# aws/s2n-quic

Measured on AMD Instinct MI355X. Metric: GiB/s AEAD seal+open, device-resident, 1200 B packets at 1/2/4/8 MI355X, higher is better.
Workload: dtype u8

## Files before the change

### s2n-quic_amd/csrc/check_resources.py

```python
import re
import sys

bad = []
for path in sys.argv[1:]:
    name = None
    for line in open(path, errors="replace"):
        m = re.search(r"remark: Function Name: (\S+)", line)
        if m:
            name = m.group(1)
            continue
        if not name:
            continue
        lds = re.search(r"LDS Size \[bytes/block\]: (\d+)", line)
        scr = re.search(r"ScratchSize \[bytes/lane\]: (\d+)", line)
        dyn_lds = any(k in name for k in ("aes_gcm_quad_kernel", "aes_gcm_quad_rx_kernel", "aes_gcm_wave_kernel",
                                          "aes_gcm_burst_kernel", "txq_server_kernel"))
        default = ("aes_gcm_wave_kernel" in name or re.search(r"aes_gcm_quad_kernelILb[01]ELi10E", name)
                   or re.search(r"aes_gcm_quad_rx_kernelILi10E", name))
        if lds and dyn_lds and int(lds.group(1)) != 0:
            bad.append(f"{name}: {lds.group(1)} B of static LDS on top of the dynamic 160 KiB")
        if scr and default and int(scr.group(1)) > 32:
            bad.append(f"{name}: {scr.group(1)} B/lane of scratch")
if bad:
    sys.exit("kernel resource check failed:\n  " + "\n  ".join(bad))
```

### s2n-quic_amd/csrc/device_common.h

```cpp
#pragma once

#include <utility>

#include "qpp_internal.h"

namespace qpp {
namespace dev {

constexpr uint32_t kLdsGhash = 0;
constexpr uint32_t kLdsAes = 65536;
constexpr uint32_t kLdsV = 131072;
constexpr uint32_t kLdsStage = 131072;
constexpr uint32_t kLdsMax = 163840;

typedef uint32_t u32x4 __attribute__((ext_vector_type(4)));
typedef __attribute__((address_space(3))) uint32_t lds_u32;
typedef __attribute__((address_space(3))) u32x4 lds_u128;
__device__ __forceinline__ uint32_t lds_ld32(uint32_t a) { return *(const lds_u32 *)(size_t)a; }
__device__ __forceinline__ uint4 lds_ld128(uint32_t a) {
    const u32x4 v = *(const lds_u128 *)(size_t)a;
    return make_uint4(v.x, v.y, v.z, v.w);
}
__device__ __forceinline__ void lds_st32(uint32_t a, uint32_t v) { *(lds_u32 *)(size_t)a = v; }
__device__ __forceinline__ uint32_t lds_add32(uint32_t a, uint32_t v) {
// ... 374 lines not shown
    const uint32_t s = d_sbox[x], s2 = xtime4(s);
    const uint32_t t0 = s2 | (s << 8) | (s << 16) | ((s2 ^ s) << 24);
    for (uint32_t d = threadIdx.x; d < 8192; d += blockDim.x) {
        const uint32_t slot = ((d >> 8) + x) & 31u, m = slot >> 3;
        lds_st32(base + 256u * x + 4u * slot, __builtin_amdgcn_alignbit(t0, t0, (32u - 8u * m) & 31u));
    }
}

#ifdef __HIP_DEVICE_COMPILE__
typedef const __attribute__((address_space(4))) uint4 *RkPtr;
#else
typedef const uint4 *RkPtr;
#endif

struct CtrPageQ4 {
    uint32_t k0, k1, k2, k3;
    uint32_t l0, l1, l2, l3;
    uint32_t x3;
    uint32_t page;

    template <typename RK>
    __device__ __forceinline__ void build(const AesQ4 &a, RK rkp, uint32_t n0, uint32_t n1, uint32_t n2, uint32_t pg) {
        const uint4 r0 = rkp[0], r1 = rkp[1], r2 = rkp[2];
        const uint32_t rk[12] = {r0.x, r0.y, r0.z, r0.w, r1.x, r1.y, r1.z, r1.w, r2.x, r2.y, r2.z, r2.w};
        build(a, rk, n0, n1, n2, pg);
    }
    __device__ __forceinline__ void build(const AesQ4 &a, const uint32_t *__restrict__ rk, uint32_t n0, uint32_t n1,
                                          uint32_t n2, uint32_t pg) {
        const uint32_t s0 = a.rot(n0 ^ rk[0]), s1 = a.rot(n1 ^ rk[1]), s2 = a.rot(n2 ^ rk[2]),
                       s3 = a.rot(bswap32(pg << 8) ^ rk[3]);
        k0 = xor3(a.look<0>(s0), a.look<1>(s1), a.look<2>(s2)) ^ a.rot(rk[4]);
        k1 = a.col(s1, s2, s3, s0, a.rot(rk[5]));
        k2 = a.col(s2, s3, s0, s1, a.rot(rk[6]));
        k3 = a.col(s3, s0, s1, s2, a.rot(rk[7]));
        l0 = xor3(a.look<1>(k1), a.look<2>(k2), a.look<3>(k3)) ^ a.rot(rk[8]);
        l1 = xor3(a.look<0>(k1), a.look<1>(k2), a.look<2>(k3)) ^ a.rot(rk[9]);
        l2 = xor3(a.look<0>(k2), a.look<1>(k3), a.look<3>(k1)) ^ a.rot(rk[10]);
        l3 = xor3(a.look<0>(k3), a.look<2>(k1), a.look<3>(k2)) ^ a.rot(rk[11]);
        x3 = rk[3] >> 24;
        page = pg;
    }
    __device__ __forceinline__ void two_rounds(const AesQ4 &a, uint32_t c, uint32_t (&v)[4]) const {
        const uint32_t u0 = k0 ^ a.lookx(c ^ x3);
        v[0] = l0 ^ a.look<0>(u0);
        v[1] = l1 ^ a.look<3>(u0);
        v[2] = l2 ^ a.look<2>(u0);
        v[3] = l3 ^ a.look<1>(u0);
    }
};

#ifndef QPP_Q4_DEPTH
#define QPP_Q4_DEPTH 3
#endif
template <int NR, int NB, int STRIDE = 1>
__device__ __forceinline__ void ctr_keystream_q4(const AesQ4 &a, const CtrPageQ4 &pg, const uint32_t *__restrict__ rk,
                                                 uint32_t c0, uint4 (&ks)[NB]) {
    static_assert(NB >= 1 && NB <= 4, "pipeline depth NB - 1 lookups groups of 4 within the 15-read counter");
    constexpr int D = NB - 1 < QPP_Q4_DEPTH ? NB - 1 : QPP_Q4_DEPTH;
    constexpr int U = (NR - 2) * 4 * NB;
    uint32_t st[NB][4];
    uint32_t nw[4];
    uint32_t kr[4];
    uint32_t ld[D + 1][4];
#pragma unroll
    for (int j = 0; j < NB; j++) pg.two_rounds(a, c0 + STRIDE * j, st[j]);
    auto issue = [&](auto uc) {
        constexpr int u = decltype(uc)::value;
        constexpr int j = (u / 4) % NB, c = u % 4;
        const uint32_t *s = st[j];
        uint32_t *l = ld[u % (D + 1)];
        l[0] = a.look<0>(s[c]);
        l[1] = a.look<1>(s[(c + 1) & 3]);
        l[2] = a.look<2>(s[(c + 2) & 3]);
        l[3] = a.look<3>(s[(c + 3) & 3]);
    };
    auto combine = [&](auto uc) {
        constexpr int u = decltype(uc)::value;
        constexpr int r = 3 + u / (4 * NB), j = (u / 4) % NB, c = u % 4;
        const uint32_t *l = ld[u % (D + 1)];
        if constexpr (u % (4 * NB) == 0) {
#pragma unroll
            for (int i = 0; i < 4; i++) kr[i] = r < NR ? a.rot(rk[4 * r + i]) : rk[4 * r + i];
        }
        if constexpr (r < NR) {
            nw[c] = AesQ4::comb(l[0], l[1], l[2], l[3], kr[c]);
        } else {
            nw[c] = a.fin(l[0], l[1], l[2], l[3], kr[c]);
        }
        if constexpr (c == 3) {
#pragma unroll
            for (int i = 0; i < 4; i++) st[j][i] = nw[i];
        }
    };
    static_for<D>([&](auto uc) { issue(uc); });
    static_for<U>([&](auto uc) {
        constexpr int u = decltype(uc)::value;
        if constexpr (u + D < U) issue(std::integral_constant<int, u + D>{});
        __builtin_amdgcn_sched_barrier(0);
        combine(uc);
        __builtin_amdgcn_sched_barrier(0);
    });
#pragma unroll
    for (int j = 0; j < NB; j++) ks[j] = make_uint4(st[j][0], st[j][1], st[j][2], st[j][3]);
}

struct PacketView {
    uint8_t *base;
    uint32_t aad_len, len, pn_len;
    uint32_t n0, n1, n2;
};

// ... 225 lines not shown
```

### s2n-quic_amd/csrc/ghash.h

```cpp
#pragma once

#include "device_common.h"

namespace qpp {
namespace dev {

#ifndef QPP_GHASH_DEPTH
#define QPP_GHASH_DEPTH 9
#endif
template <bool PIPE>
struct GhashT {
    uint32_t lc[4];
    uint32_t sel[4];
    bool q1, q2;

    __device__ __forceinline__ static GhashT make() {
        GhashT g;
        const uint32_t r = threadIdx.x & 15u, q = r >> 2, b = r & 3u;
#pragma unroll
        for (int k = 0; k < 4; k++) {
            uint32_t v = 0;
#pragma unroll
            for (int i = 0; i < 4; i++) v |= ((4u * ((k + q) & 3u) + ((i + b) & 3u)) << 4) << (8 * i);
            g.lc[k] = v;
        }
#pragma unroll
        for (int i = 0; i < 4; i++) g.sel[i] = 0x0c0c0000u | ((4u + ((i + b) & 3u)) << 8) | (uint32_t)i;
        g.q1 = q & 1u;
        g.q2 = (q >> 1) & 1u;
        return g;
    }
    __device__ __forceinline__ uint4 rot(uint4 z) const {
        const uint4 a = q1 ? make_uint4(z.y, z.z, z.w, z.x) : z;
        return q2 ? make_uint4(a.z, a.w, a.x, a.y) : a;
    }
    template <int K, int I>
    __device__ __forceinline__ uint4 look(const uint4 &w) const {
        const uint32_t wk = K == 0 ? w.x : K == 1 ? w.y : K == 2 ? w.z : w.w;
        return lds_ld128(kLdsGhash + __builtin_amdgcn_perm(wk, lc[K], sel[I]));
    }
    __device__ __forceinline__ uint4 prod(const uint4 &w, uint4 c) const {
        if constexpr (!PIPE) {
            const uint4 a = xor3(look<0, 0>(w), look<0, 1>(w), look<0, 2>(w));
            const uint4 b = xor3(look<0, 3>(w), look<1, 0>(w), look<1, 1>(w));
            const uint4 d = xor3(look<1, 2>(w), look<1, 3>(w), look<2, 0>(w));
            const uint4 e = xor3(look<2, 1>(w), look<2, 2>(w), look<2, 3>(w));
            const uint4 f = xor3(look<3, 0>(w), look<3, 1>(w), look<3, 2>(w));
            const uint4 g = xor3(a, b, d);
            const uint4 h = xor3(e, f, look<3, 3>(w));
            return xor3(g, h, c);
        }
        if constexpr (QPP_GHASH_DEPTH != 9) return prod_d<QPP_GHASH_DEPTH>(w, c);
        uint4 l[16];
        auto issue = [&](auto ic) {
            constexpr int i = decltype(ic)::value;
            l[i] = look<i / 4, i % 4>(w);
        };
        static_for<9>(issue);
        __builtin_amdgcn_sched_barrier(0);
        const uint4 a = xor3(l[0], l[1], l[2]);
        issue(std::integral_constant<int, 9>{});
        issue(std::integral_constant<int, 10>{});
        issue(std::integral_constant<int, 11>{});
        __builtin_amdgcn_sched_barrier(0);
        const uint4 b = xor3(l[3], l[4], l[5]);
        issue(std::integral_constant<int, 12>{});
        issue(std::integral_constant<int, 13>{});
        issue(std::integral_constant<int, 14>{});
        __builtin_amdgcn_sched_barrier(0);
        const uint4 d = xor3(l[6], l[7], l[8]);
        issue(std::integral_constant<int, 15>{});
        __builtin_amdgcn_sched_barrier(0);
        const uint4 g = xor3(a, b, d);
        const uint4 e = xor3(l[9], l[10], l[11]);
        const uint4 f = xor3(l[12], l[13], l[14]);
        const uint4 h = xor3(e, f, l[15]);
        return xor3(g, h, c);
    }
    template <int D>
    __device__ __forceinline__ uint4 prod_d(const uint4 &w, uint4 c) const {
        uint4 l[16], x[5];
        auto issue = [&](auto ic) {
            constexpr int i = decltype(ic)::value;
            if constexpr (i < 16) l[i] = look<i / 4, i % 4>(w);
        };
        static_for<D>(issue);
        static_for<5>([&](auto tc) {
            constexpr int t = decltype(tc)::value;
            __builtin_amdgcn_sched_barrier(0);
            x[t] = xor3(l[3 * t], l[3 * t + 1], l[3 * t + 2]);
            issue(std::integral_constant<int, 3 * t + D>{});
            issue(std::integral_constant<int, 3 * t + D + 1>{});
            issue(std::integral_constant<int, 3 * t + D + 2>{});
        });
        __builtin_amdgcn_sched_barrier(0);
        return xor3(xor3(x[0], x[1], x[2]), xor3(x[3], x[4], l[15]), c);
    }
    __device__ __forceinline__ uint4 mulx(const uint4 &w, uint4 c) const { return rot(prod(w, c)); }
};
using Ghash = GhashT<false>;

__device__ inline void build_tables(const DevKey *__restrict__ key) {
    const uint32_t tid = threadIdx.x, nthr = blockDim.x;
    for (uint32_t i = tid; i < 128; i += nthr) {
        const uint32_t *v = key->V[i];
        lds_st128(kLdsV + 16 * i, make_uint4(v[0], v[1], v[2], v[3]));
    }
    build_aes_tables(kLdsAes);
    __syncthreads();
    for (uint32_t e = tid; e < 4096; e += nthr) {
        const uint32_t j = e & 15, x = e >> 4;
        uint4 acc = make_uint4(0, 0, 0, 0);
#pragma unroll
        for (int i = 0; i < 8; i++)
            if ((x >> (7 - i)) & 1) acc = acc ^ lds_ld128(kLdsV + 16 * (8 * j + i));
        lds_st128(kLdsGhash + 256 * x + 16 * j, acc);
    }
    __syncthreads();
}

template <uint32_t BASE = kLdsGhash>
struct Ghash4T {
    Ghash g;
    uint32_t hi_or, lo_or;
    __device__ __forceinline__ static Ghash4T make(uint32_t wave) {
        Ghash4T h;
        h.g = Ghash::make();
        h.hi_or = 0x01010101u * ((2u * wave + 0u) << 4);
        h.lo_or = 0x01010101u * ((2u * wave + 1u) << 4);
        return h;
    }
    __device__ __forceinline__ uint4 rot(uint4 z) const { return g.rot(z); }
    template <int K, int I>
    __device__ __forceinline__ uint4 look(uint32_t wk) const {
        return lds_ld128(BASE + __builtin_amdgcn_perm(wk, g.lc[K], g.sel[I]));
    }
    __device__ __forceinline__ uint4 prod(const uint4 &w, uint4 c) const { return prod_impl<true>(w, c); }
    __device__ __forceinline__ uint4 prod(const uint4 &w) const { return prod_impl<false>(w, w); }
    template <bool C>
    __device__ __forceinline__ uint4 prod_impl(const uint4 &w, uint4 c) const {
        const uint32_t wk[4] = {w.x, w.y, w.z, w.w};
        uint32_t hs[4], ls[4];
#pragma unroll
        for (int k = 0; k < 4; k++) {
            hs[k] = __builtin_amdgcn_bitop3_b32(wk[k] >> 4, 0x0f0f0f0fu, hi_or, 0xea);
            ls[k] = __builtin_amdgcn_bitop3_b32(wk[k], 0x0f0f0f0fu, lo_or, 0xea);
        }
        uint4 r[32];
        auto issue = [&](auto ic) {
// ... 44 lines not shown
```

### s2n-quic_amd/csrc/quad.hip

```cpp
#include <stdlib.h>

#include "device_common.h"
#include "ghash.h"

namespace qpp {
namespace {
using namespace dev;

constexpr uint32_t kQLdsPow = 131072;
constexpr uint32_t kQLdsVe = 65536;
#ifndef QPP_QUAD_WG
#define QPP_QUAD_WG 768
#endif
#ifndef QPP_QUAD_WG256
#define QPP_QUAD_WG256 768
#endif
using QAes = AesQ4;
using QPage = CtrPageQ4;
__device__ __forceinline__ QAes make_qaes() { return AesQ4::make(); }
__device__ __forceinline__ void build_qaes() { build_aes_tables_q4(kLdsAes); }
template <int NR, int NB, int STRIDE>
__device__ __forceinline__ void qkeystream(const QAes &a, const QPage &pg, RkPtr rkp, uint32_t c0,
                                           uint4 (&ks)[NB]) {
    uint32_t rk[4 * (NR + 1)];
#pragma unroll
    for (int r = 3; r <= NR; r++) {
        const uint4 v = rkp[r];
        rk[4 * r] = v.x; rk[4 * r + 1] = v.y; rk[4 * r + 2] = v.z; rk[4 * r + 3] = v.w;
    }
    ctr_keystream_q4<NR, NB, STRIDE>(a, pg, rk, c0, ks);
}
__device__ __forceinline__ uint4 ld_payload(const uint8_t *p) { return ld16(p); }
#ifndef QPP_QUAD_NT
#define QPP_QUAD_NT 1
#endif
__device__ __forceinline__ void st_payload(uint8_t *p, uint4 v) {
    if (QPP_QUAD_NT) st16_nt(p, v);
    else st16(p, v);
}
template <int NR>
constexpr int kQuadWG = NR == 14 ? QPP_QUAD_WG256 : QPP_QUAD_WG;
#ifndef QPP_QUAD_NB
#define QPP_QUAD_NB 4
#endif
#ifndef QPP_QUAD_TRACE
#ifndef QPP_QUAD_PRIO
#define QPP_QUAD_PRIO 2
#endif
#ifndef QPP_QUAD_PRIO_DROP
#define QPP_QUAD_PRIO_DROP 0
#endif
#define QPP_QUAD_TRACE 0
#endif
#ifndef QPP_QUAD_EK0C
#define QPP_QUAD_EK0C 1
#endif
#ifndef QPP_QUAD_TAGEARLY
#define QPP_QUAD_TAGEARLY 1
#endif
#ifndef QPP_QUAD_ABL
#define QPP_QUAD_ABL 0
#endif
constexpr int kQNB = QPP_QUAD_NB, kQSG = 4 * kQNB;
static_assert(kQNB >= 2 && kQNB <= 4, "group size");


__device__ __forceinline__ uint4 mul_h8(uint4 x) {
    const uint32_t w[4] = {x.x, x.y, x.z, x.w};
    uint4 acc = make_uint4(0, 0, 0, 0);
#pragma unroll
    for (int j = 0; j < 16; j++) acc = acc ^ lds_ld128(256u * ((w[j >> 2] >> (8 * (j & 3))) & 0xffu) + 16u * j);
    return acc;
}
__device__ __forceinline__ void build8(uint32_t v) {
    for (uint32_t e = threadIdx.x; e < 4096; e += blockDim.x) {
        const uint32_t j = e & 15, x = e >> 4;
        uint4 acc = make_uint4(0, 0, 0, 0);
#pragma unroll
        for (int i = 0; i < 8; i++)
            if ((x >> (7 - i)) & 1) acc = acc ^ lds_ld128(v + 16 * (8 * j + i));
        lds_st128(256 * x + 16 * j, acc);
    }
}

__device__ void quad_tables_pow(const DevKey *__restrict__ key, const uint4 *__restrict__ src) {
    const uint32_t tid = threadIdx.x, nthr = blockDim.x;
    for (uint32_t idx = tid; idx < 4 * 512; idx += nthr) {
        const uint32_t t = idx >> 9, ent = idx & 511u, pos = ent >> 4, n = ent & 15u, b = pos >> 1, h = pos & 1u;
        uint4 v;
        uint32_t e;
        if (t == 0) {
            e = 1;
            const uint4 *V = (const uint4 *)key->V;
            v = make_uint4(0, 0, 0, 0);
// ... 51 lines not shown
    return (uint32_t)__builtin_amdgcn_mov_dpp((int)v, CTRL, 0xf, 0xf, false);
}
template <int CTRL>
__device__ __forceinline__ uint4 qperm(uint4 v) {
    return make_uint4(qperm<CTRL>(v.x), qperm<CTRL>(v.y), qperm<CTRL>(v.z), qperm<CTRL>(v.w));
}
constexpr int kQuadSwap1 = 0xb1;
constexpr int kQuadSwap2 = 0x4e;
constexpr int kQuadBcast0 = 0x00;
constexpr int kQuadBcast1 = 0x55;
constexpr int kQuadBcast2 = 0xaa;

constexpr int kQuadRot1 = 0x39;
constexpr int kQuadRot3 = 0x93;
#ifndef QPP_QUAD_HPS
#define QPP_QUAD_HPS 1
#endif
template <int NR>
__device__ __forceinline__ uint32_t aes_quad(const QAes &a, const uint32_t *__restrict__ rk_g, uint32_t col, uint32_t s) {
    uint32_t rk[NR + 1];
    RkPtr hp{};
    if (QPP_QUAD_HPS) {
        uint64_t p = (uint64_t)rk_g;
        asm volatile("" : "+s"(p));
        hp = (RkPtr)p;
    } else {
#pragma unroll
        for (int r = 0; r <= NR; r++) rk[r] = rk_g[4 * r + s];
    }
    auto rkey = [&](int r) {
        if (!QPP_QUAD_HPS) return rk[r];
        const uint4 v = hp[r];
        return s == 0 ? v.x : s == 1 ? v.y : s == 2 ? v.z : v.w;
    };
    uint32_t x = a.rot(col ^ rkey(0));
#pragma unroll
    for (int r = 1; r <= NR; r++) {
        const uint32_t b = qperm<kQuadRot1>(x), c = qperm<kQuadSwap2>(x), d = qperm<kQuadRot3>(x);
        if (r < NR) {
            x = a.col(x, b, c, d, a.rot(rkey(r)));
        } else {
            x = a.last(x, b, c, d, rkey(r));
        }
    }
    return x;
}

__device__ __forceinline__ qpp_pkt reload_desc(const qpp_pkt *descs, uint32_t i) {
    uint32_t v = i;
    asm volatile("" : "+v"(v));
    return descs[v];
}

template <int NR, bool SEAL, bool HEAD>
__device__ __forceinline__ void quad_packet(const QAes &aes, const GhashT<true> &gh, const DevKey *__restrict__ key,
                                            bool has, const qpp_pkt &d,
                                            const qpp_pkt *__restrict__ descs, uint32_t pkt_index,
                                            uint8_t *__restrict__ arena, uint8_t *masks, int8_t *status,
                                            uint32_t flags, uint32_t s) {
    const uint32_t aad_len = d.aad_len, len = has ? d.pt_len : 0u, pay = d.off + aad_len;
    const uint32_t pn_len = SEAL ? (uint32_t)d.pn_len : 0u;
    constexpr bool kLatePro = !SEAL || NR == 10;
    uint32_t iv0, iv1, iv2;
    if constexpr (kLatePro) {
        uint64_t iva = (uint64_t)key->iv;
        asm volatile("" : "+s"(iva));
        const __attribute__((address_space(4))) uint32_t *ivp = (const __attribute__((address_space(4))) uint32_t *)iva;
        iv0 = ivp[0]; iv1 = ivp[1]; iv2 = ivp[2];
    } else {
        iv0 = key->iv[0]; iv1 = key->iv[1]; iv2 = key->iv[2];
    }
    const uint32_t n0 = iv0, n1 = iv1 ^ bswap32((uint32_t)(d.pn >> 32)), n2 = iv2 ^ bswap32((uint32_t)d.pn);
    const int nfull = (int)(len >> 4), rem = (int)(len & 15), m = nfull + (rem ? 1 : 0);
    const int a = has ? (int)((aad_len + 15) >> 4) : 0;
    auto at = [&](uint32_t off) { return arena + off; };

    auto round_keys = [&]() {
        uint64_t a = (uint64_t)key->rk;
        asm volatile("" : "+s"(a));
        return (RkPtr)a;
    };
    QPage pg;
    uint32_t z0;
    asm volatile("v_mov_b32 %0, 0" : "=v"(z0));
    uint4 w = make_uint4(z0, z0, z0, z0);
    {
        auto aad_block = [&](int t) {
            const uint32_t i = (uint32_t)(t + a - 1);
            uint4 x = ld16(at(d.off + 16 * i));
            const uint32_t r = aad_len - 16 * i;
            return r < 16 ? keep_bytes(x, r) : x;
        };
        int t = (1 - a) + (((int)s - (1 - a)) & 3);
        const bool has_aad = t <= 0;
        const uint32_t i0 = (uint32_t)(t + a - 1), r0 = aad_len - 16 * i0;
        if constexpr (!kLatePro) {
            if (has_aad) {
                w = gh.rot(aad_block(t));
                t += 4;
            }
        }
        const uint4 x0 = kLatePro ? ld16(at(d.off + (has_aad ? 16 * i0 : 0u))) : make_uint4(z0, z0, z0, z0);
        pg.build(aes, round_keys(), n0, n1, n2, 0);
        if (kLatePro && has_aad) {
            w = gh.rot(r0 < 16 ? keep_bytes(x0, r0) : x0);
            t += 4;
        }
        for (; t <= 0; t += 4) w = gh.mulx(w, aad_block(t));
    }

    const int ngroups = has ? (m + kQSG) / kQSG : 0;
    const int G = (int)wave_max((uint32_t)ngroups);
    const int min_full = (int)__builtin_amdgcn_readfirstlane(wave_min(has ? (uint32_t)nfull : 0u));
    auto interior = [&](int g) { return g >= 1 && kQSG * g + kQSG - 1 <= min_full; };
    const bool head_ok = HEAD && kQSG - 1 <= min_full;
    const int tail_slots = (int)wave_max(has ? (uint32_t)max(0, m + 1 - kQSG * (G - 1)) : 0u);
    auto lenblk = [&]() { return make_uint4(0, bswap32(aad_len * 8), 0, bswap32(len * 8)); };
    bool len_done = !has;

    constexpr int HNR = NR == 10 ? 10 : 14;
    const bool want_hp = SEAL && (flags & (QPP_HP_MASK_OUT | QPP_HP_APPLY)) != 0;
    uint4 ek0 = make_uint4(0, 0, 0, 0);
    uint32_t ek0c = 0;

    bool hp_done = false;
    const bool hp_at0 = want_hp && has && pn_len >= 1 && pn_len <= 4 && len + pn_len >= 20;
    HdrBytes hb{0u, 0u};
    auto hp_early = [&](const uint4 &ct) {
        if (!hp_at0) return;
        const uint4 b0 = qperm<kQuadBcast1>(ct), b1 = qperm<kQuadBcast2>(ct);
        const uint32_t lo = s == 0 ? b0.x : s == 1 ? b0.y : s == 2 ? b0.z : b0.w;
        const uint32_t hi = s == 0 ? b0.y : s == 1 ? b0.z : s == 2 ? b0.w : b1.x;
        const uint32_t col = __builtin_amdgcn_alignbyte(hi, lo, 4 - pn_len);
        const uint32_t m0 = aes_quad<HNR>(aes, key->hp_rk, col, s);
        const uint32_t m1 = qperm<kQuadBcast1>(m0);
        if (s == 0) {
            if (flags & QPP_HP_MASK_OUT) {
                uint8_t *mo = masks + 5 * (size_t)pkt_index;
                mo[0] = (uint8_t)m0; mo[1] = (uint8_t)(m0 >> 8); mo[2] = (uint8_t)(m0 >> 16);
                mo[3] = (uint8_t)(m0 >> 24); mo[4] = (uint8_t)m1;
            }
            const uint32_t hdr_len = aad_len - pn_len;
            if (flags & QPP_HP_APPLY) hdr_apply(at(pay - aad_len), hdr_len, pn_len, hb, m0, m1);
        }
        hp_done = true;
    };

    auto group = [&](auto nbc, int g) __attribute__((always_inline)) {
        constexpr int NBG = decltype(nbc)::value;
        const bool head = NBG == kQNB && g == 0 && head_ok;
        const bool inner = NBG == kQNB && interior(g);
        const RkPtr rkp = round_keys();
        const int t0 = kQSG * g + (int)s;
        uint4 ks[NBG];
        uint4 in[NBG];
        const uint32_t c0 = (uint32_t)t0 + 1u;
        uint32_t m0 = n0, m1 = n1, m2 = n2;
        if (((kQSG * g + 1) >> 8) == ((kQSG * g + kQSG) >> 8)) {
            if ((c0 >> 8) != pg.page) {
                asm volatile("" : "+v"(m0), "+v"(m1), "+v"(m2));
                pg.build(aes, rkp, m0, m1, m2, c0 >> 8);
            }
            qkeystream<NR, NBG, 4>(aes, pg, rkp, c0, ks);
        } else {
            asm volatile("" : "+v"(m0), "+v"(m1), "+v"(m2));
            uint32_t rk[4 * (NR + 1)];
#pragma unroll
            for (int r = 0; r <= NR; r++) {
                const uint4 v = rkp[r];
                rk[4 * r] = v.x; rk[4 * r + 1] = v.y; rk[4 * r + 2] = v.z; rk[4 * r + 3] = v.w;
            }
            static_for<NBG>([&](auto kc) {
                constexpr int k = decltype(kc)::value;
                ks[k] = aes.encrypt<NR>(make_uint4(m0, m1, m2, bswap32(c0 + 4 * k)), rk);
            });
        }
        if (QPP_QUAD_PRIO) __builtin_amdgcn_s_setprio(QPP_QUAD_PRIO);
        if (SEAL && g == 0 && hp_at0 && (flags & QPP_HP_APPLY) && s == 0) hb = hdr_load(at(pay - aad_len), aad_len - pn_len);
        if (head) {
            const uint32_t b = pay + 16 * (uint32_t)(t0 - 1);
#pragma unroll
            for (int k = 0; k < NBG; k++) in[k] = ld_payload(at(k == 0 && s == 0 ? pay : b + 64 * k));
        } else if (inner) {
            const uint32_t b = pay + 16 * (uint32_t)(t0 - 1);
#pragma unroll
            for (int k = 0; k < NBG; k++) {
                if (QPP_QUAD_ABL & 1) in[k] = make_uint4(b + k, b ^ k, b, k);
                else in[k] = ld_payload(at(b + 64 * k));
            }
        } else {
#pragma unroll
            for (int k = 0; k < NBG; k++) {
                const int j = t0 + 4 * k - 1;
                in[k] = ld_payload(at(pay + (j >= 0 && 16 * j <= (int)len ? 16 * (uint32_t)j : 0u)));
            }
        }
        uint4 out[NBG];
#pragma unroll
        for (int k = 0; k < NBG; k++) out[k] = in[k] ^ ks[k];
        if constexpr (SEAL) {
            if (g == 0 && !QPP_QUAD_EK0C) ek0 = ks[0];
        }
        if (QPP_QUAD_EK0C && g == 0) {
            const uint32_t c0w = qperm<kQuadBcast0>(ks[0].x), c1w = qperm<kQuadBcast0>(ks[0].y),
                           c2w = qperm<kQuadBcast0>(ks[0].z), c3w = qperm<kQuadBcast0>(ks[0].w);
            ek0c = s == 0 ? c0w : s == 1 ? c1w : s == 2 ? c2w : c3w;
        }
        if (head) {
            const uint32_t b = pay + 16 * (uint32_t)(t0 - 1);
#pragma unroll
            for (int k = 0; k < NBG; k++)
                if (k != 0 || s != 0) st_payload(at(b + 64 * k), out[k]);
#pragma unroll
            for (int k = 0; k < NBG; k++) {
                const uint4 wn = gh.mulx(w, SEAL ? out[k] : in[k]);
                if (k != 0) {
                    w = wn;
                } else {
                    w.x = s != 0 ? wn.x : w.x;
                    w.y = s != 0 ? wn.y : w.y;
                    w.z = s != 0 ? wn.z : w.z;
                    w.w = s != 0 ? wn.w : w.w;
                }
            }
        } else if (inner) {
            const uint32_t b = pay + 16 * (uint32_t)(t0 - 1);
#pragma unroll
            for (int k = 0; k < NBG; k++)
                if (!(QPP_QUAD_ABL & 2)) st_payload(at(b + 64 * k), out[k]);
            if (QPP_QUAD_PRIO && QPP_QUAD_PRIO_DROP == 1) __builtin_amdgcn_s_setprio(0);
#pragma unroll
            for (int k = 0; k < NBG; k++) w = gh.mulx(w, SEAL ? out[k] : in[k]);
        } else {
            uint32_t rl = (uint32_t)rem;
            asm volatile("" : "+v"(rl));
#pragma unroll
            for (int k = 0; k < NBG; k++) {
                const int t = t0 + 4 * k, j = t - 1;
                const bool full = t >= 1 && j < nfull, part = rem && j == nfull, lenslot = has && t == m + 1;
                if (full) st_payload(at(pay + 16 * (uint32_t)j), out[k]);
                if (part) st_bytes(at(pay + 16 * (uint32_t)j), keep_bytes(out[k], rl), rl);
                const uint4 x = lenslot ? lenblk() : part ? keep_bytes(SEAL ? out[k] : in[k], rl)
                                                        : (SEAL ? out[k] : in[k]);
                if (full || part || lenslot) w = gh.mulx(w, x);
                len_done = len_done || lenslot;
            }
        }
        if (SEAL && g == 0 && !(QPP_QUAD_ABL & 4)) hp_early(out[0]);
        if (QPP_QUAD_PRIO) __builtin_amdgcn_s_setprio(0);
    };
    for (int g = 0; g + 1 < G; g++) group(std::integral_constant<int, kQNB>{}, g);
    uint32_t want = 0;
    if (!SEAL && QPP_QUAD_TAGEARLY) __builtin_memcpy(&want, at(pay + len + 4 * s), 4);
    if (G > 0) {
        if (tail_slots <= 4) group(std::integral_constant<int, 1>{}, G - 1);
        else if (kQNB == 2 || tail_slots <= 8) group(std::integral_constant<int, 2>{}, G - 1);
        else if (kQNB == 3 || tail_slots <= 12) group(std::integral_constant<int, kQNB < 3 ? kQNB : 3>{}, G - 1);
        else group(std::integral_constant<int, kQNB>{}, G - 1);
    }
    if (!len_done && (((m + 1) & 3) == (int)s)) w = gh.mulx(w, lenblk());
    const int t_last = (m + 1) - (((m + 1) - (int)s) & 3);
    const uint32_t e = (uint32_t)(m + 2 - t_last);
    Ghash4T<kQLdsPow> fin;
    for (int k = 0; k < 4; k++) {
        fin.g.lc[k] = gh.lc[k];
        fin.g.sel[k] = gh.sel[k];
    }
    fin.g.q1 = gh.q1;
    fin.g.q2 = gh.q2;
    fin.hi_or = 0x01010101u * ((2u * (e - 1u)) << 4);
    fin.lo_or = 0x01010101u * ((2u * (e - 1u) + 1u) << 4);
    uint4 y = (QPP_QUAD_ABL & 8) ? w : fin.prod(w);
    y = y ^ qperm<kQuadSwap1>(y);
    y = y ^ qperm<kQuadSwap2>(y);

    if constexpr (SEAL) {
        if (QPP_QUAD_EK0C) {
            const uint32_t t = (s == 0 ? y.x : s == 1 ? y.y : s == 2 ? y.z : y.w) ^ ek0c;
            if (has) __builtin_memcpy(at(pay + len + 4 * s), &t, 4);
        } else if (has && s == 0) {
            st16(at(pay + len), y ^ ek0);
        }
        const bool hp = !(QPP_QUAD_ABL & 4) && want_hp && has && pn_len >= 1 && pn_len <= 4 && len >= 4 - pn_len;
        if (hp && !hp_done) {
            __builtin_amdgcn_fence(__ATOMIC_SEQ_CST, "wavefront");
            uint32_t col;
            __builtin_memcpy(&col, at(pay + 4 - pn_len + 4 * s), 4);
            const uint32_t m0 = aes_quad<HNR>(aes, key->hp_rk, col, s);
            const uint32_t m1 = qperm<kQuadBcast1>(m0);
            if (s == 0) {
                if (flags & QPP_HP_MASK_OUT) {
                    uint8_t *mo = masks + 5 * (size_t)pkt_index;
                    mo[0] = (uint8_t)m0; mo[1] = (uint8_t)(m0 >> 8); mo[2] = (uint8_t)(m0 >> 16);
                    mo[3] = (uint8_t)(m0 >> 24); mo[4] = (uint8_t)m1;
                }
                const uint32_t hdr_len = aad_len - pn_len;
                if (flags & QPP_HP_APPLY) hdr_apply(at(pay - aad_len), hdr_len, pn_len, hdr_load(at(pay - aad_len), hdr_len), m0, m1);
            }
        }
        if (!has || s != 0) return;
        if (status) status[pkt_index] = want_hp && !hp ? QPP_DECODE_ERROR : QPP_OK;
    } else {
        uint32_t ek0 = ek0c;
        if (!QPP_QUAD_EK0C) {
            const qpp_pkt dt = reload_desc(descs, pkt_index);
            const uint32_t j0 = s == 0 ? key->iv[0]
                              : s == 1 ? key->iv[1] ^ bswap32((uint32_t)(dt.pn >> 32))
                              : s == 2 ? key->iv[2] ^ bswap32((uint32_t)dt.pn)
                                       : bswap32(1u);
            uint32_t sl = s;
            asm volatile("" : "+v"(sl));
            ek0 = aes_quad<NR>(aes, key->rk, j0, sl);
        }
        if (!QPP_QUAD_TAGEARLY) __builtin_memcpy(&want, at(pay + len + 4 * s), 4);
        const uint32_t ys = s == 0 ? y.x : s == 1 ? y.y : s == 2 ? y.z : y.w;
        uint32_t diff = ys ^ ek0 ^ want;
        diff |= qperm<kQuadSwap1>(diff);
        diff |= qperm<kQuadSwap2>(diff);
        if (!has || s != 0) return;
        const bool ok = diff == 0;
        if (!ok) {
            __builtin_amdgcn_fence(__ATOMIC_SEQ_CST, "wavefront");
            for (int b = 0; b < nfull; b++) st16(at(pay + 16 * b), make_uint4(0, 0, 0, 0));
            if (rem) st_bytes(at(pay + 16 * nfull), make_uint4(0, 0, 0, 0), (uint32_t)rem);
        }
        status[pkt_index] = ok ? QPP_OK : QPP_DECRYPT_ERROR;
    }
}

template <bool SEAL, int NR, int WG = kQuadWG<NR>, bool HEAD = false>
__device__ __forceinline__ void quad_slices(const DevKey *__restrict__ keys, const qpp_pkt *__restrict__ descs,
                                            const uint32_t *__restrict__ perm, const WorkItem *__restrict__ work,
                                            const uint32_t *__restrict__ meta, uint8_t *__restrict__ arena,
                                            uint8_t *masks, int8_t *status, uint32_t flags, uint32_t single,
                                            uint32_t n_single, const PowTables pow, uint32_t fix_lo = 0,
                                            uint32_t fix_hi = 0) {
    const bool one = single != 0xffffffffu;
    uint32_t i_lo = 0, i_hi = 1, p0 = 0, n = n_single;
    if (!one) {
        const uint32_t items = meta[0], i10 = meta[1], n10 = meta[2], n14 = meta[3];
        i_lo = NR == 10 ? 0 : i10;
        i_hi = NR == 10 ? i10 : items;
        p0 = NR == 10 ? 0 : n10;
        n = NR == 10 ? n10 : n14;
    }
    const uint32_t P = ((n + gridDim.x - 1) / gridDim.x + 15u) & ~15u;
    uint32_t lo = fix_hi ? fix_lo : p0 + min(n, blockIdx.x * P);
    const uint32_t hi = fix_hi ? fix_hi : p0 + min(n, (blockIdx.x + 1) * P);
    if (lo >= hi) return;
    uint32_t i = i_lo, j = i_hi;
    while (!one && j - i > 1) {
        const uint32_t mid = (i + j) >> 1;
        if (work[mid].begin <= lo) i = mid; else j = mid;
    }
    const QAes aes = make_qaes();
    const GhashT<true> gh = GhashT<true>::make();
    const uint32_t s = threadIdx.x & 3u, q = threadIdx.x >> 2;
    build_qaes();
#if QPP_QUAD_TRACE
    uint64_t t_beg = __builtin_amdgcn_s_memtime(), t_tab = 0, r_beg = __builtin_amdgcn_s_memrealtime();
    uint32_t n_seg = 0;
#endif
    for (; lo < hi; i++) {
        WorkItem w = one ? WorkItem{single, 0u, n, (uint32_t)NR} : work[i];
        w.key = __builtin_amdgcn_readfirstlane(w.key);
        w.begin = __builtin_amdgcn_readfirstlane(w.begin);
        w.count = __builtin_amdgcn_readfirstlane(w.count);
        const uint32_t end = min(hi, w.begin + w.count);
        const DevKey *__restrict__ key = keys + w.key;
        __syncthreads();
#if QPP_QUAD_TRACE
        const uint64_t t0 = __builtin_amdgcn_s_memtime();
#endif
        if (w.key < pow.cap) quad_tables_pow(key, (const uint4 *)(pow.base + (size_t)w.key * kPowBytes));
        else quad_tables(key);
#if QPP_QUAD_TRACE
        t_tab += __builtin_amdgcn_s_memtime() - t0;
        n_seg++;
#endif
        for (uint32_t t0 = lo; t0 < end; t0 += WG / 4) {
            const uint32_t t = t0 + q;
            const bool real = t < end;
            const uint32_t pi = one ? (real ? t : lo) : perm[real ? t : lo];
            const qpp_pkt d = descs[pi];
            bool has = real && !(d.flags & QPP_PKT_SKIP);
            if (one && has && d.key_idx != single) {
                if (status && s == 0) status[pi] = QPP_INTERNAL_ERROR;
                has = false;
            }
            quad_packet<NR, SEAL, HEAD>(aes, gh, key, has, d, descs, pi, arena, masks, status, flags, s);
        }
        lo = end;
    }
#if QPP_QUAD_TRACE
    __syncthreads();
    if (threadIdx.x == 0 && (QPP_QUAD_TRACE == 2 || blockIdx.x == 0 || blockIdx.x == gridDim.x / 2))
        printf("quad wg %u seal %d nr %d: %u segments, tables %llu of %llu cycles, real %llu-%llu\n", blockIdx.x,
               (int)SEAL, NR, n_seg, (unsigned long long)t_tab, (unsigned long long)(__builtin_amdgcn_s_memtime() - t_beg),
               (unsigned long long)r_beg, (unsigned long long)__builtin_amdgcn_s_memrealtime());
#endif
}

template <bool SEAL, int NR>
__global__ __launch_bounds__(kQuadWG<NR>) void aes_gcm_quad_kernel(const DevKey *__restrict__ keys,
                                                              const qpp_pkt *__restrict__ descs,
                                                              const uint32_t *__restrict__ perm,
                                                              const WorkItem *__restrict__ work,
                                                              const uint32_t *__restrict__ meta,
                                                              uint8_t *__restrict__ arena, uint8_t *masks,
                                                              int8_t *status, uint32_t flags, uint32_t single,
                                                              uint32_t n_single, const PowTables pow) {
    constexpr int WG = kQuadWG<NR>;
    if constexpr (NR != 14) quad_slices<SEAL, 10, WG, NR == 10>(keys, descs, perm, work, meta, arena, masks, status, flags, single, n_single, pow);
    if constexpr (NR != 10) quad_slices<SEAL, 14, WG>(keys, descs, perm, work, meta, arena, masks, status, flags, single, n_single, pow);
}

#ifndef QPP_RX_TRACE
#define QPP_RX_TRACE 0
#endif
constexpr uint32_t kRxCtl = kQLdsPow;
constexpr uint32_t kRxCls = kRxCtl + 1024;
typedef __attribute__((address_space(3))) uint8_t lds_u8;
constexpr uint32_t kRxHistMax = 16384;
constexpr uint64_t kRxBarrierTicks = 100000000ull;
constexpr int8_t kRxOpen = 0x7f;

constexpr uint32_t kRxLocal = kRxCtl + 8;

__device__ uint32_t rx_arrive(uint32_t *ctr) {
    __syncthreads();
    if (threadIdx.x == 0) {
        __builtin_amdgcn_fence(__ATOMIC_RELEASE, "agent");
        const uint32_t old = __hip_atomic_fetch_add(ctr, 1u, __ATOMIC_RELAXED, __HIP_MEMORY_SCOPE_AGENT);
        __builtin_amdgcn_fence(__ATOMIC_ACQUIRE, "agent");
        lds_st32(kRxCtl, old);
    }
    __syncthreads();
    return lds_ld32(kRxCtl);
}

__device__ bool rx_wait(uint32_t *scratch, uint32_t *ctr, uint32_t target) {
    __syncthreads();
    if (threadIdx.x == 0) {
        uint32_t ok = 1;
        const uint64_t t0 = __builtin_amdgcn_s_memrealtime();
        while (__hip_atomic_load(ctr, __ATOMIC_RELAXED, __HIP_MEMORY_SCOPE_AGENT) < target) {
            if (__hip_atomic_load(&scratch[1], __ATOMIC_RELAXED, __HIP_MEMORY_SCOPE_AGENT) ||
                __builtin_amdgcn_s_memrealtime() - t0 > kRxBarrierTicks) {
                __hip_atomic_store(&scratch[1], 1u, __ATOMIC_RELAXED, __HIP_MEMORY_SCOPE_AGENT);
                ok = 0;
                break;
            }
            __builtin_amdgcn_s_sleep(2);
        }
        __builtin_amdgcn_fence(__ATOMIC_ACQUIRE, "agent");
        lds_st32(kRxCtl, ok);
    }
    __syncthreads();
    return lds_ld32(kRxCtl) != 0;
}

__device__ __forceinline__ uint32_t rx_class(uint4 kw, bool chacha) {
    if (kw.w != 1) return 3u;
    if (kw.x == QPP_SUITE_TLS_CHACHA20_POLY1305_SHA256) return chacha ? 2u : 3u;
    return kw.y == 10 ? 0u : kw.y == 14 ? 1u : 3u;
}

template <int AES>
constexpr int kRxWG = AES == 14 ? kQuadWG<14> : kQuadWG<10>;
template <int AES>
__global__ __launch_bounds__(kRxWG<AES>) void aes_gcm_quad_rx_kernel(const DevKey *__restrict__ keys,
                                                                 uint32_t key_cap, const qpp_rx_pkt *__restrict__ rx,
                                                                 uint32_t n, uint8_t *arena, qpp_pkt *descs_out,
                                                                 int8_t *status, uint32_t *scratch, uint32_t *perm,
                                                                 uint32_t *timeouts, uint32_t chacha, const PowTables pow) {
    uint32_t *counts = scratch + 16, *cursor = counts + key_cap, *meta = cursor + key_cap;
    WorkItem *work = (WorkItem *)(meta + 4);
#if QPP_RX_TRACE
    uint64_t ts[8] = {};
    ts[0] = __builtin_amdgcn_s_memrealtime();
#define RX_TS(i) ts[i] = __builtin_amdgcn_s_memrealtime()
#else
#define RX_TS(i) (void)0
#endif
    const uint32_t tid = threadIdx.x, nt = blockDim.x;
    const uint32_t bins = min(key_cap, kRxHistMax);
    build_qaes();
    for (uint32_t i = tid; i < bins; i += nt) lds_st32(4 * i, 0);
    if (tid == 0) lds_st32(kRxLocal, 0xffffffffu);
    __syncthreads();
    const QAes aes = make_qaes();
    RX_TS(1);
    const uint32_t P = (n + gridDim.x - 1) / gridDim.x;
    const uint32_t lo = min(n, blockIdx.x * P), hi = min(n, lo + P);
    qpp_rx_pkt r_next = lo + tid < hi ? rx[lo + tid] : qpp_rx_pkt{};
    for (uint32_t t = lo + tid; t < hi; t += nt) {
        const qpp_rx_pkt r = r_next;
        if (t + nt < hi) r_next = rx[t + nt];
        uint4 kw;
        const qpp_pkt d = rx_unprotect_one(aes, keys, key_cap, r, arena, status, t, &kw);
        if (!(d.flags & QPP_PKT_SKIP)) {
            const uint32_t cls = rx_class(kw, chacha != 0);
            if (cls < 3) {
                status[t] = kRxOpen;
                lds_add32(4 * d.key_idx, 1u);
            } else if (!(kw.w == 1 && kw.x == QPP_SUITE_TLS_CHACHA20_POLY1305_SHA256)) {
                status[t] = QPP_INTERNAL_ERROR;
            }
        }
        descs_out[t] = d;
    }
    auto bail = [&]() {
        if (tid == 0) __hip_atomic_fetch_add(timeouts, 1u, __ATOMIC_RELAXED, __HIP_MEMORY_SCOPE_AGENT);
        for (uint32_t t = lo + tid; t < hi; t += nt)
            if (status[t] == kRxOpen) status[t] = QPP_INTERNAL_ERROR;
    };
    __syncthreads();
    for (uint32_t k = tid; k < bins; k += nt) {
        const uint32_t c = lds_ld32(4 * k);
        if (c && c == hi - lo) {
            const uint32_t cls = rx_class(*(const uint4 *)(keys + k), chacha != 0);
            if ((cls == 0 && AES != 14) || (cls == 1 && AES != 10)) {
// ... 166 lines not shown
```

Measured before the change: 1065.

## Run AES-128 quad kernel at 1024 threads with lighter GHASH and peeled first group

Raises the AES-128 quad seal/open workgroup from 768 to 1024 threads, aiming for four waves per SIMD. To fit the tighter register budget it uses a shallower GHASH lookup pipeline with a running-accumulator reduction, and makes the Q4 keystream depth configurable. It also peels the first group out of the packet loop so first-group checks resolve at compile time, and pins the thread offset in a register. The rx kernel keeps its 768-thread size, and a resource check now enforces the occupancy target. Less memory-latency hiding per wave and possible spills are the risks.

```diff
diff --git a/s2n-quic_amd/csrc/check_resources.py b/s2n-quic_amd/csrc/check_resources.py
--- a/s2n-quic_amd/csrc/check_resources.py
+++ b/s2n-quic_amd/csrc/check_resources.py
@@ -1,7 +1,11 @@
 import re
 import sys
 
+SCRATCH_MAX = 32
+QUAD128_WAVES = 4
+
 bad = []
+seen128 = set()
 for path in sys.argv[1:]:
     name = None
     for line in open(path, errors="replace"):
@@ -17,9 +21,17 @@
                                           "aes_gcm_burst_kernel", "txq_server_kernel"))
         default = ("aes_gcm_wave_kernel" in name or re.search(r"aes_gcm_quad_kernelILb[01]ELi10E", name)
                    or re.search(r"aes_gcm_quad_rx_kernelILi10E", name))
+        quad128 = re.search(r"aes_gcm_quad_kernelILb([01])ELi10E", name)
+        occ = re.search(r"Occupancy \[waves/SIMD\]: (\d+)", line)
+        if occ and quad128:
+            seen128.add(quad128.group(1))
+            if int(occ.group(1)) != QUAD128_WAVES:
+                bad.append(f"{name}: occupancy {occ.group(1)} waves/SIMD, not {QUAD128_WAVES}")
         if lds and dyn_lds and int(lds.group(1)) != 0:
             bad.append(f"{name}: {lds.group(1)} B of static LDS on top of the dynamic 160 KiB")
-        if scr and default and int(scr.group(1)) > 32:
+        if scr and default and int(scr.group(1)) > SCRATCH_MAX:
             bad.append(f"{name}: {scr.group(1)} B/lane of scratch")
+if any(p.endswith("quad.res") for p in sys.argv[1:]) and seen128 != {"0", "1"}:
+    bad.append("quad.res: no occupancy remark for the AES-128 quad seal / open pair")
 if bad:
     sys.exit("kernel resource check failed:\n  " + "\n  ".join(bad))
diff --git a/s2n-quic_amd/csrc/device_common.h b/s2n-quic_amd/csrc/device_common.h
--- a/s2n-quic_amd/csrc/device_common.h
+++ b/s2n-quic_amd/csrc/device_common.h
@@ -450,11 +450,11 @@
 #ifndef QPP_Q4_DEPTH
 #define QPP_Q4_DEPTH 3
 #endif
-template <int NR, int NB, int STRIDE = 1>
+template <int NR, int NB, int STRIDE = 1, int DEPTH = QPP_Q4_DEPTH>
 __device__ __forceinline__ void ctr_keystream_q4(const AesQ4 &a, const CtrPageQ4 &pg, const uint32_t *__restrict__ rk,
                                                  uint32_t c0, uint4 (&ks)[NB]) {
     static_assert(NB >= 1 && NB <= 4, "pipeline depth NB - 1 lookups groups of 4 within the 15-read counter");
-    constexpr int D = NB - 1 < QPP_Q4_DEPTH ? NB - 1 : QPP_Q4_DEPTH;
+    constexpr int D = NB - 1 < DEPTH ? NB - 1 : DEPTH;
     constexpr int U = (NR - 2) * 4 * NB;
     uint32_t st[NB][4];
     uint32_t nw[4];
diff --git a/s2n-quic_amd/csrc/ghash.h b/s2n-quic_amd/csrc/ghash.h
--- a/s2n-quic_amd/csrc/ghash.h
+++ b/s2n-quic_amd/csrc/ghash.h
@@ -8,7 +8,7 @@
 #ifndef QPP_GHASH_DEPTH
 #define QPP_GHASH_DEPTH 9
 #endif
-template <bool PIPE>
+template <bool PIPE, int DEPTH = QPP_GHASH_DEPTH, bool ACC = false>
 struct GhashT {
     uint32_t lc[4];
     uint32_t sel[4];
@@ -50,7 +50,8 @@
             const uint4 h = xor3(e, f, look<3, 3>(w));
             return xor3(g, h, c);
         }
-        if constexpr (QPP_GHASH_DEPTH != 9) return prod_d<QPP_GHASH_DEPTH>(w, c);
+        if constexpr (ACC) return prod_acc<DEPTH>(w, c);
+        if constexpr (DEPTH != 9) return prod_d<DEPTH>(w, c);
         uint4 l[16];
         auto issue = [&](auto ic) {
             constexpr int i = decltype(ic)::value;
@@ -95,6 +96,26 @@
         });
         __builtin_amdgcn_sched_barrier(0);
         return xor3(xor3(x[0], x[1], x[2]), xor3(x[3], x[4], l[15]), c);
+    }
+    template <int D>
+    __device__ __forceinline__ uint4 prod_acc(const uint4 &w, uint4 c) const {
+        static_assert(D % 2 == 0 && D >= 2 && D <= 16, "reads are consumed in pairs");
+        uint4 l[16];
+        auto issue = [&](auto ic) {
+            constexpr int i = decltype(ic)::value;
+            if constexpr (i < 16) l[i] = look<i / 4, i % 4>(w);
+        };
+        static_for<D>(issue);
+        uint4 acc = c;
+        static_for<8>([&](auto tc) {
+            constexpr int t = decltype(tc)::value;
+            __builtin_amdgcn_sched_barrier(0);
+            acc = xor3(acc, l[2 * t], l[2 * t + 1]);
+            issue(std::integral_constant<int, 2 * t + D>{});
+            issue(std::integral_constant<int, 2 * t + D + 1>{});
+        });
+        __builtin_amdgcn_sched_barrier(0);
+        return acc;
     }
     __device__ __forceinline__ uint4 mulx(const uint4 &w, uint4 c) const { return rot(prod(w, c)); }
 };
diff --git a/s2n-quic_amd/csrc/quad.hip b/s2n-quic_amd/csrc/quad.hip
--- a/s2n-quic_amd/csrc/quad.hip
+++ b/s2n-quic_amd/csrc/quad.hip
@@ -9,6 +9,9 @@
 
 constexpr uint32_t kQLdsPow = 131072;
 constexpr uint32_t kQLdsVe = 65536;
+#ifndef QPP_QUAD_WG128
+#define QPP_QUAD_WG128 1024
+#endif
 #ifndef QPP_QUAD_WG
 #define QPP_QUAD_WG 768
 #endif
@@ -19,7 +22,7 @@
 using QPage = CtrPageQ4;
 __device__ __forceinline__ QAes make_qaes() { return AesQ4::make(); }
 __device__ __forceinline__ void build_qaes() { build_aes_tables_q4(kLdsAes); }
-template <int NR, int NB, int STRIDE>
+template <int NR, int NB, int STRIDE, int DEPTH>
 __device__ __forceinline__ void qkeystream(const QAes &a, const QPage &pg, RkPtr rkp, uint32_t c0,
                                            uint4 (&ks)[NB]) {
     uint32_t rk[4 * (NR + 1)];
@@ -28,7 +31,7 @@
         const uint4 v = rkp[r];
         rk[4 * r] = v.x; rk[4 * r + 1] = v.y; rk[4 * r + 2] = v.z; rk[4 * r + 3] = v.w;
     }
-    ctr_keystream_q4<NR, NB, STRIDE>(a, pg, rk, c0, ks);
+    ctr_keystream_q4<NR, NB, STRIDE, DEPTH>(a, pg, rk, c0, ks);
 }
 __device__ __forceinline__ uint4 ld_payload(const uint8_t *p) { return ld16(p); }
 #ifndef QPP_QUAD_NT
@@ -39,7 +42,29 @@
     else st16(p, v);
 }
 template <int NR>
-constexpr int kQuadWG = NR == 14 ? QPP_QUAD_WG256 : QPP_QUAD_WG;
+constexpr int kQuadWG = NR == 10 ? QPP_QUAD_WG128 : NR == 14 ? QPP_QUAD_WG256 : QPP_QUAD_WG;
+#ifndef QPP_QUAD4_GHASH_DEPTH
+#define QPP_QUAD4_GHASH_DEPTH 6
+#endif
+#ifndef QPP_QUAD4_GHASH_ACC
+#define QPP_QUAD4_GHASH_ACC 1
+#endif
+#ifndef QPP_QUAD4_PEEL
+#define QPP_QUAD4_PEEL 1
+#endif
+#ifndef QPP_QUAD4_Q4_DEPTH
+#define QPP_QUAD4_Q4_DEPTH QPP_Q4_DEPTH
+#endif
+template <int WG>
+struct QuadCfg {
+    static constexpr bool four = WG > 768;
+    static constexpr int gh_depth = four ? QPP_QUAD4_GHASH_DEPTH : QPP_GHASH_DEPTH;
+    static constexpr int q4_depth = four ? QPP_QUAD4_Q4_DEPTH : QPP_Q4_DEPTH;
+    static constexpr bool peel = four && QPP_QUAD4_PEEL;
+    using Gh = GhashT<true, gh_depth, four && QPP_QUAD4_GHASH_ACC>;
+};
+static_assert(kQuadWG<10> % 256 == 0 && kQuadWG<14> % 256 == 0 && kQuadWG<0> % 256 == 0 && kQuadWG<10> <= 1024,
+              "build_aes_tables_q4 needs whole 256-thread rows");
 #ifndef QPP_QUAD_NB
 #define QPP_QUAD_NB 4
 #endif
@@ -197,8 +222,8 @@
     return descs[v];
 }
 
-template <int NR, bool SEAL, bool HEAD>
-__device__ __forceinline__ void quad_packet(const QAes &aes, const GhashT<true> &gh, const DevKey *__restrict__ key,
+template <int NR, bool SEAL, bool HEAD, typename CFG>
+__device__ __forceinline__ void quad_packet(const QAes &aes, const typename CFG::Gh &gh, const DevKey *__restrict__ key,
                                             bool has, const qpp_pkt &d,
                                             const qpp_pkt *__restrict__ descs, uint32_t pkt_index,
                                             uint8_t *__restrict__ arena, uint8_t *masks, int8_t *status,
@@ -291,10 +316,11 @@
         hp_done = true;
     };
 
-    auto group = [&](auto nbc, int g) __attribute__((always_inline)) {
-        constexpr int NBG = decltype(nbc)::value;
-        const bool head = NBG == kQNB && g == 0 && head_ok;
-        const bool inner = NBG == kQNB && interior(g);
+    auto group = [&](auto nbc, int g, auto fc) __attribute__((always_inline)) {
+        constexpr int NBG = decltype(nbc)::value, F = decltype(fc)::value;
+        const bool first = F < 0 ? g == 0 : F == 1;
+        const bool head = NBG == kQNB && first && head_ok;
+        const bool inner = NBG == kQNB && !(F == 1) && interior(g);
         const RkPtr rkp = round_keys();
         const int t0 = kQSG * g + (int)s;
         uint4 ks[NBG];
@@ -306,7 +332,7 @@
                 asm volatile("" : "+v"(m0), "+v"(m1), "+v"(m2));
                 pg.build(aes, rkp, m0, m1, m2, c0 >> 8);
             }
-            qkeystream<NR, NBG, 4>(aes, pg, rkp, c0, ks);
+            qkeystream<NR, NBG, 4, CFG::q4_depth>(aes, pg, rkp, c0, ks);
         } else {
             asm volatile("" : "+v"(m0), "+v"(m1), "+v"(m2));
             uint32_t rk[4 * (NR + 1)];
@@ -320,8 +346,10 @@
                 ks[k] = aes.encrypt<NR>(make_uint4(m0, m1, m2, bswap32(c0 + 4 * k)), rk);
             });
         }
+        int tg = t0;
+        if constexpr (CFG::four) asm volatile("" : "+v"(tg));
         if (QPP_QUAD_PRIO) __builtin_amdgcn_s_setprio(QPP_QUAD_PRIO);
-        if (SEAL && g == 0 && hp_at0 && (flags & QPP_HP_APPLY) && s == 0) hb = hdr_load(at(pay - aad_len), aad_len - pn_len);
+        if (SEAL && first && hp_at0 && (flags & QPP_HP_APPLY) && s == 0) hb = hdr_load(at(pay - aad_len), aad_len - pn_len);
         if (head) {
             const uint32_t b = pay + 16 * (uint32_t)(t0 - 1);
 #pragma unroll
@@ -336,7 +364,7 @@
         } else {
 #pragma unroll
             for (int k = 0; k < NBG; k++) {
-                const int j = t0 + 4 * k - 1;
+                const int j = tg + 4 * k - 1;
                 in[k] = ld_payload(at(pay + (j >= 0 && 16 * j <= (int)len ? 16 * (uint32_t)j : 0u)));
             }
         }
@@ -344,9 +372,9 @@
 #pragma unroll
         for (int k = 0; k < NBG; k++) out[k] = in[k] ^ ks[k];
         if constexpr (SEAL) {
-            if (g == 0 && !QPP_QUAD_EK0C) ek0 = ks[0];
-        }
-        if (QPP_QUAD_EK0C && g == 0) {
+            if (first && !QPP_QUAD_EK0C) ek0 = ks[0];
+        }
+        if (QPP_QUAD_EK0C && first) {
             const uint32_t c0w = qperm<kQuadBcast0>(ks[0].x), c1w = qperm<kQuadBcast0>(ks[0].y),
                            c2w = qperm<kQuadBcast0>(ks[0].z), c3w = qperm<kQuadBcast0>(ks[0].w);
             ek0c = s == 0 ? c0w : s == 1 ? c1w : s == 2 ? c2w : c3w;
@@ -381,7 +409,7 @@
             asm volatile("" : "+v"(rl));
 #pragma unroll
             for (int k = 0; k < NBG; k++) {
-                const int t = t0 + 4 * k, j = t - 1;
+                const int t = tg + 4 * k, j = t - 1;
                 const bool full = t >= 1 && j < nfull, part = rem && j == nfull, lenslot = has && t == m + 1;
                 if (full) st_payload(at(pay + 16 * (uint32_t)j), out[k]);
                 if (part) st_bytes(at(pay + 16 * (uint32_t)j), keep_bytes(out[k], rl), rl);
@@ -391,18 +419,35 @@
                 len_done = len_done || lenslot;
             }
         }
-        if (SEAL && g == 0 && !(QPP_QUAD_ABL & 4)) hp_early(out[0]);
+        if (SEAL && first && !(QPP_QUAD_ABL & 4)) hp_early(out[0]);
         if (QPP_QUAD_PRIO) __builtin_amdgcn_s_setprio(0);
     };
-    for (int g = 0; g + 1 < G; g++) group(std::integral_constant<int, kQNB>{}, g);
+    using Unknown = std::integral_constant<int, -1>;
+    using NotFirst = std::integral_constant<int, CFG::peel ? 0 : -1>;
+    using First = std::integral_constant<int, CFG::peel ? 1 : -1>;
+    if constexpr (CFG::peel) {
+        if (G > 1) group(std::integral_constant<int, kQNB>{}, 0, First{});
+        for (int g = 1; g + 1 < G; g++) group(std::integral_constant<int, kQNB>{}, g, NotFirst{});
+    } else {
+        for (int g = 0; g + 1 < G; g++) group(std::integral_constant<int, kQNB>{}, g, Unknown{});
+    }
     uint32_t want = 0;
     if (!SEAL && QPP_QUAD_TAGEARLY) __builtin_memcpy(&want, at(pay + len + 4 * s), 4);
-    if (G > 0) {
-        if (tail_slots <= 4) group(std::integral_constant<int, 1>{}, G - 1);
-        else if (kQNB == 2 || tail_slots <= 8) group(std::integral_constant<int, 2>{}, G - 1);
-        else if (kQNB == 3 || tail_slots <= 12) group(std::integral_constant<int, kQNB < 3 ? kQNB : 3>{}, G - 1);
-        else group(std::integral_constant<int, kQNB>{}, G - 1);
-    }
+#define QPP_LAST_GROUP(FC)                                                                                      \
+    do {                                                                                                        \
+        if (tail_slots <= 4) group(std::integral_constant<int, 1>{}, G - 1, FC{});                              \
+        else if (kQNB == 2 || tail_slots <= 8) group(std::integral_constant<int, 2>{}, G - 1, FC{});            \
+        else if (kQNB == 3 || tail_slots <= 12)                                                                 \
+            group(std::integral_constant<int, kQNB < 3 ? kQNB : 3>{}, G - 1, FC{});                             \
+        else group(std::integral_constant<int, kQNB>{}, G - 1, FC{});                                           \
+    } while (0)
+    if constexpr (CFG::peel) {
+        if (G == 1) QPP_LAST_GROUP(First);
+        else if (G > 1) QPP_LAST_GROUP(NotFirst);
+    } else {
+        if (G > 0) QPP_LAST_GROUP(Unknown);
+    }
+#undef QPP_LAST_GROUP
     if (!len_done && (((m + 1) & 3) == (int)s)) w = gh.mulx(w, lenblk());
     const int t_last = (m + 1) - (((m + 1) - (int)s) & 3);
     const uint32_t e = (uint32_t)(m + 2 - t_last);
@@ -499,7 +544,8 @@
         if (work[mid].begin <= lo) i = mid; else j = mid;
     }
     const QAes aes = make_qaes();
-    const GhashT<true> gh = GhashT<true>::make();
+    using CFG = QuadCfg<WG>;
+    const typename CFG::Gh gh = CFG::Gh::make();
     const uint32_t s = threadIdx.x & 3u, q = threadIdx.x >> 2;
     build_qaes();
 #if QPP_QUAD_TRACE
@@ -533,7 +579,7 @@
                 if (status && s == 0) status[pi] = QPP_INTERNAL_ERROR;
                 has = false;
             }
-            quad_packet<NR, SEAL, HEAD>(aes, gh, key, has, d, descs, pi, arena, masks, status, flags, s);
+            quad_packet<NR, SEAL, HEAD, CFG>(aes, gh, key, has, d, descs, pi, arena, masks, status, flags, s);
         }
         lo = end;
     }
@@ -612,7 +658,7 @@
 }
 
 template <int AES>
-constexpr int kRxWG = AES == 14 ? kQuadWG<14> : kQuadWG<10>;
+constexpr int kRxWG = AES == 14 ? kQuadWG<14> : kQuadWG<0>;
 template <int AES>
 __global__ __launch_bounds__(kRxWG<AES>) void aes_gcm_quad_rx_kernel(const DevKey *__restrict__ keys,
                                                                  uint32_t key_cap, const qpp_rx_pkt *__restrict__ rx,
```

After: 1079, median of 6. 1.01x the previous value.
